# 3SAILab/two_stage_object_detection

Measured on AMD Instinct MI355X. Metric: images/sec Faster R-CNN ResNet-50 @800x1333, higher is better.
Workload: dtype f32 storage/accumulate; conv products as bf16x3 (3 exact bf16 pieces per operand, 6 bf16 MFMAs per product) in 0 of 43 conv layers, as fp16x2 (2 fp16 pieces of 2^e x per operand, 3 fp16 MFMAs per product; e follows the tensor's abs-max per forward: range words) in 43, f32 MFMA in the rest; 1 GPU; Full Faster R-CNN resnet50 inference forward, batch=1 per GPU, 3x800x1333, 80+1 classes, 3000->300 proposals; global_batch=1, parallelism=dp1, hip_graph=True, autotuned_tiles=True, steps_in_flight=4, tiles_tuned_on=this rank

## Files before the change

### two_stage_object_detection_amd/csrc/bottleneck_fused.hip

```cpp
#include "tsod_internal.h"
#include <type_traits>

namespace {

typedef float f32x16 __attribute__((ext_vector_type(16)));
typedef unsigned int u32x4 __attribute__((ext_vector_type(4)));

constexpr int TW = 16, HW_ = TW + 2;
constexpr int CMID = 64;
constexpr int Y_PITCH = 144;
constexpr int W_STEP = 8192;
template <int TH> struct Geo {
    static constexpr int HALO = (TH + 2) * (TW + 2);
    static constexpr int PB1 = (HALO + 31) / 32, PB2 = TH * TW / 32;
    static constexpr int Y_PLANE = PB1 * 32 * Y_PITCH;
    static constexpr int A_PLANE = PB1 * 32 * 64, A_STAGE = 2 * A_PLANE;
    static constexpr int Y_BYTES = 2 * Y_PLANE, SCR_OFF = Y_BYTES, LDS_BYTES = SCR_OFF + 64;
    static_assert(TH * TW % 32 == 0 && 2 * A_STAGE <= Y_BYTES && 2 * LDS_BYTES <= 160 * 1024, "x stages inside the y region; two workgroups per CU");
};
constexpr unsigned kOOB = 0xFFFFFFF0u;

struct Params {
    const float *x;
    float *out;
    const unsigned char *wstream;
    const float *bn;
    int N, H, W, Cin, in_pitch, Cout, out_pitch;
    int tiles_x, tiles_y;
    unsigned x_bytes, out_bytes;
    float slope;
    int w_exp1, w_exp2, w_exp3;
    float a_scale;
    const unsigned *amax_in;
    unsigned *amax_out;
    int *range_flag;
};

__device__ __forceinline__ int off64(int row, int slot) { return row * 64 + ((slot ^ ((row >> 2) & 3)) << 4); }

__device__ __forceinline__ float4 bload4(__amdgpu_buffer_rsrc_t r, unsigned off) {
    const u32x4 v = __builtin_amdgcn_raw_buffer_load_b128(r, off, 0, 0);
    return make_float4(__uint_as_float(v.x), __uint_as_float(v.y), __uint_as_float(v.z), __uint_as_float(v.w));
}

struct WFrag { u32x4 h[2], l[2]; };
struct AFrag { u32x4 h, l; };

template <int TH, bool PROJ = false>
__global__ void __launch_bounds__(256, 2) bottleneck_kernel(const Params p) {
    using G = Geo<TH>;
    constexpr int HALO = G::HALO, PB1 = G::PB1, PB2 = G::PB2, Y_PLANE = G::Y_PLANE, A_PLANE = G::A_PLANE, A_STAGE = G::A_STAGE,
                  SCR_OFF = G::SCR_OFF, LDS_BYTES = G::LDS_BYTES;
    __shared__ __align__(16) unsigned char lds[LDS_BYTES];
    const int tid = threadIdx.x, lane = tid & 63, wave = tid >> 6;
    const int j = lane & 31, hh = lane >> 5;
    const int cb = wave & 1, pb0 = wave >> 1;
    const int nb1 = (PB1 - pb0 + 1) / 2, nb2 = (PB2 - pb0 + 1) / 2;
    float *scr = reinterpret_cast<float *>(lds + SCR_OFF);

    const int tiles_per_img = p.tiles_x * p.tiles_y;
    const int nwg = (int)gridDim.x, per = nwg >> 3, r8 = nwg & 7, xcd = (int)blockIdx.x & 7;
    const int tile_id = (xcd < r8 ? xcd * (per + 1) : r8 * (per + 1) + (xcd - r8) * per) + ((int)blockIdx.x >> 3);
    const int img = tile_id / tiles_per_img, t_in = tile_id - img * tiles_per_img;
    const int ty = t_in / p.tiles_x, tx = t_in - ty * p.tiles_x;
    const int h0 = ty * TH, w0 = tx * TW;
    const __amdgpu_buffer_rsrc_t rs_x = __builtin_amdgcn_make_buffer_rsrc((void *)p.x, (short)0, (int)p.x_bytes, 0x00020000);
    const __amdgpu_buffer_rsrc_t rs_o = __builtin_amdgcn_make_buffer_rsrc((void *)p.out, (short)0, (int)p.out_bytes, 0x00020000);

    float a_scale = p.a_scale;
    int e_x;
    if (p.amax_in != nullptr) {
        e_x = tsod_fp16x2_exp_from_bits(tsod_amax_reduce_bits(p.amax_in[lane * TSOD_AMAX_STRIDE_WORDS]));
        a_scale = __uint_as_float((unsigned)(127 + e_x) << 23);
    } else {
        e_x = (int)(__float_as_uint(a_scale) >> 23) - 127;
    }
    a_scale = __uint_as_float((unsigned)__builtin_amdgcn_readfirstlane((int)__float_as_uint(a_scale)));

    const int n_steps1 = p.Cin / 32, sps = PROJ ? 2 + n_steps1 : 2, n_steps = n_steps1 + 18 + (p.Cout / 64) * sps;
    const u32x4 *wbase = reinterpret_cast<const u32x4 *>(p.wstream + cb * (W_STEP / 2) + lane * 64);
    auto w_load = [&](int s, WFrag &f) {
        if (s >= n_steps) return;
        const u32x4 *src = wbase + (size_t)s * (W_STEP / 16);
        f.h[0] = src[0]; f.l[0] = src[1]; f.h[1] = src[2]; f.l[1] = src[3];
    };
    WFrag wf[3];
    w_load(0, wf[0]);
    w_load(1, wf[1]);

    constexpr int NX = PB1;
    unsigned xoff[NX];
    int xdst[NX];
#pragma unroll
    for (int i = 0; i < NX; ++i) {
        const int u = tid + 256 * i, row = u >> 3, q = u & 7;
        const int hr = row / HW_, hc = row - hr * HW_;
        const int gh = h0 - 1 + hr, gw = w0 - 1 + hc;
        const bool ok = row < HALO && (unsigned)gh < (unsigned)p.H && (unsigned)gw < (unsigned)p.W;
        xoff[i] = ok ? (unsigned)((((long)img * p.H + gh) * p.W + gw) * p.in_pitch + q * 4) * 4u : kOOB;
        xdst[i] = off64(row, q >> 1) + (q & 1) * 8;
    }
    float4 xr[NX];
    auto x_load = [&](int ks) {
        if (ks >= n_steps1) return;
#pragma unroll
        for (int i = 0; i < NX; ++i) xr[i] = bload4(rs_x, xoff[i] != kOOB ? xoff[i] + (unsigned)ks * 128u : kOOB);
    };
    auto x_store = [&](int stage) {
#pragma unroll
        for (int i = 0; i < NX; ++i) {
            unsigned h0_, l0_, h1_, l1_;
            tsod_split2_pair(xr[i].x, xr[i].y, a_scale, h0_, l0_);
            tsod_split2_pair(xr[i].z, xr[i].w, a_scale, h1_, l1_);
            *reinterpret_cast<uint2 *>(lds + stage * A_STAGE + xdst[i]) = make_uint2(h0_, h1_);
            *reinterpret_cast<uint2 *>(lds + stage * A_STAGE + A_PLANE + xdst[i]) = make_uint2(l0_, l1_);
        }
    };
    int xfa[4][2];
#pragma unroll
    for (int b = 0; b < 4; ++b)
#pragma unroll
        for (int c = 0; c < 2; ++c) xfa[b][c] = off64((pb0 + 2 * b) * 32 + j, 2 * c + hh);

    f32x16 acc[4];
#pragma unroll
    for (int b = 0; b < 4; ++b)
#pragma unroll
        for (int e = 0; e < 16; ++e) acc[b][e] = 0.f;
    x_load(0);
    x_store(0);
    x_load(1);
    __syncthreads();
    auto conv1_step = [&](auto STAGE, int ks) {
        constexpr int stage = decltype(STAGE)::value;
        w_load(ks + 2, wf[2]);
        if (ks + 1 < n_steps1) x_store(stage ^ 1);
        x_load(ks + 2);
#pragma unroll
        for (int c = 0; c < 2; ++c) {
#pragma unroll
            for (int b = 0; b < 4; ++b) {
                if (b < nb1) {
                    const u32x4 ah = *reinterpret_cast<const u32x4 *>(lds + xfa[b][c] + stage * A_STAGE);
                    const u32x4 al = *reinterpret_cast<const u32x4 *>(lds + xfa[b][c] + stage * A_STAGE + A_PLANE);
                    tsod_mfma3(acc[b], wf[0].h[c], wf[0].l[c], ah, al);
                }
            }
        }
        wf[0] = wf[1];
        wf[1] = wf[2];
        __syncthreads();
    };
    for (int ks = 0; ks < n_steps1; ks += 2) {
        conv1_step(std::integral_constant<int, 0>{}, ks);
        conv1_step(std::integral_constant<int, 1>{}, ks + 1);
    }
    const int ch16 = cb * 32 + 16 * hh;
    const float sc1 = __uint_as_float((unsigned)(127 - e_x - p.w_exp1) << 23);
    float mx = 0.f, chk = 0.f;
    {
        float sv[16], bv[16];
#pragma unroll
        for (int v = 0; v < 4; ++v) {
            const float4 s4 = *reinterpret_cast<const float4 *>(p.bn + ch16 + 4 * v), b4 = *reinterpret_cast<const float4 *>(p.bn + 64 + ch16 + 4 * v);
            sv[4 * v] = s4.x * sc1; sv[4 * v + 1] = s4.y * sc1; sv[4 * v + 2] = s4.z * sc1; sv[4 * v + 3] = s4.w * sc1;
            bv[4 * v] = b4.x; bv[4 * v + 1] = b4.y; bv[4 * v + 2] = b4.z; bv[4 * v + 3] = b4.w;
        }
#pragma unroll
        for (int b = 0; b < 4; ++b) {
            if (b >= nb1) continue;
            const int row = (pb0 + 2 * b) * 32 + j, hr = row / HW_, hc = row - hr * HW_;
            const bool ok = row < HALO && (unsigned)(h0 - 1 + hr) < (unsigned)p.H && (unsigned)(w0 - 1 + hc) < (unsigned)p.W;
            const float keep = ok ? 1.f : 0.f;
#pragma unroll
            for (int e = 0; e < 16; ++e) {
                chk = fmaf(acc[b][e], 0.f, chk);
                const float v = keep * tsod_prelu(fmaf(acc[b][e], sv[e], bv[e]), p.slope);
                acc[b][e] = v;
                mx = fmaxf(mx, fabsf(v));
            }
        }
    }
    mx = tsod_block_max(mx, scr, tid);
    const int e1 = tsod_fp16x2_exp_from_bits(__float_as_uint(mx));
    const float ys1 = __uint_as_float((unsigned)(127 + e1) << 23);
    auto y_store = [&](const f32x16 &v, int row, float ysc) {
        unsigned hq[8], lq[8];
#pragma unroll
        for (int e = 0; e < 8; ++e) tsod_split2_pair(v[2 * e], v[2 * e + 1], ysc, hq[e], lq[e]);
        unsigned char *dst = lds + (row * Y_PITCH + (4 * cb + 2 * hh) * 16);
        *reinterpret_cast<u32x4 *>(dst) = u32x4{hq[0], hq[1], hq[2], hq[3]};
        *reinterpret_cast<u32x4 *>(dst + 16) = u32x4{hq[4], hq[5], hq[6], hq[7]};
        *reinterpret_cast<u32x4 *>(dst + Y_PLANE) = u32x4{lq[0], lq[1], lq[2], lq[3]};
        *reinterpret_cast<u32x4 *>(dst + Y_PLANE + 16) = u32x4{lq[4], lq[5], lq[6], lq[7]};
    };
#pragma unroll
    for (int b = 0; b < 4; ++b)
        if (b < nb1) y_store(acc[b], (pb0 + 2 * b) * 32 + j, ys1);
    __syncthreads();

    int yfa[3];
#pragma unroll
    for (int b = 0; b < 3; ++b) {
        int pidx = (pb0 + 2 * b) * 32 + j;
        pidx = pidx < TH * TW ? pidx : TH * TW - 1;
        yfa[b] = ((pidx / TW) * HW_ + (pidx % TW)) * Y_PITCH + hh * 16;
    }
#pragma unroll
    for (int b = 0; b < 3; ++b)
#pragma unroll
        for (int e = 0; e < 16; ++e) acc[b][e] = 0.f;
    const int s2base = n_steps1;
    AFrag af[2][3];
    auto y1_frags = [&](int n, AFrag (&f)[3]) {
        const int t = n >> 1, c = n & 1, tap = t >> 1, kh = tap / 3, kw = tap - kh * 3;
        const int imm = (kh * HW_ + kw) * Y_PITCH + (t & 1) * 64 + c * 32;
#pragma unroll
        for (int b = 0; b < 3; ++b)
            if (b < nb2) {
                f[b].h = *reinterpret_cast<const u32x4 *>(lds + yfa[b] + imm);
                f[b].l = *reinterpret_cast<const u32x4 *>(lds + yfa[b] + imm + Y_PLANE);
            }
    };
    y1_frags(0, af[0]);
#pragma unroll
    for (int t = 0; t < 18; ++t) {
        w_load(s2base + t + 2, wf[(t + 2) % 3]);
#pragma unroll
        for (int c = 0; c < 2; ++c) {
            const int n = 2 * t + c;
            if (n + 1 < 36) y1_frags(n + 1, af[(n + 1) & 1]);
#pragma unroll
            for (int b = 0; b < 3; ++b)
                if (b < nb2) tsod_mfma3(acc[b], wf[t % 3].h[c], wf[t % 3].l[c], af[n & 1][b].h, af[n & 1][b].l);
            __builtin_amdgcn_sched_barrier(0);
        }
    }
    __syncthreads();
    const float sc2 = __uint_as_float((unsigned)(127 - e1 - p.w_exp2) << 23);
    mx = 0.f;
    {
        float sv[16], bv[16];
#pragma unroll
        for (int v = 0; v < 4; ++v) {
            const float4 s4 = *reinterpret_cast<const float4 *>(p.bn + 128 + ch16 + 4 * v), b4 = *reinterpret_cast<const float4 *>(p.bn + 192 + ch16 + 4 * v);
            sv[4 * v] = s4.x * sc2; sv[4 * v + 1] = s4.y * sc2; sv[4 * v + 2] = s4.z * sc2; sv[4 * v + 3] = s4.w * sc2;
            bv[4 * v] = b4.x; bv[4 * v + 1] = b4.y; bv[4 * v + 2] = b4.z; bv[4 * v + 3] = b4.w;
        }
#pragma unroll
        for (int b = 0; b < 3; ++b) {
            if (b >= nb2) continue;
#pragma unroll
            for (int e = 0; e < 16; ++e) {
                chk = fmaf(acc[b][e], 0.f, chk);
                const float v = tsod_prelu(fmaf(acc[b][e], sv[e], bv[e]), p.slope);
                acc[b][e] = v;
                mx = fmaxf(mx, fabsf(v));
            }
        }
    }
    mx = tsod_block_max(mx, scr, tid);
    const int e2 = tsod_fp16x2_exp_from_bits(__float_as_uint(mx));
    const float ys2 = __uint_as_float((unsigned)(127 + e2) << 23);
#pragma unroll
    for (int b = 0; b < 3; ++b)
        if (b < nb2) y_store(acc[b], (pb0 + 2 * b) * 32 + j, ys2);
    __syncthreads();

    const float sc3 = __uint_as_float((unsigned)(127 - e2 - p.w_exp3) << 23);
    float amax = 0.f;
    constexpr int P_PITCH = 144, P_BYTES = 32 * P_PITCH;
    static_assert(2 * P_BYTES <= Y_PLANE - TH * TW * Y_PITCH, "two patches per gap of the y region");
    unsigned char *patch = lds + (wave >> 1) * Y_PLANE + TH * TW * Y_PITCH + (wave & 1) * P_BYTES;
    const int ep_px = lane >> 3, ep_q = lane & 7;
    int y2a[3];
    unsigned xpix[3][4], opix[3][4];
#pragma unroll
    for (int b = 0; b < 3; ++b) {
        const int pidx = (pb0 + 2 * b) * 32 + j;
        y2a[b] = (pidx < TH * TW ? pidx : TH * TW - 1) * Y_PITCH + hh * 16;
#pragma unroll
        for (int i = 0; i < 4; ++i) {
            const int pe = (pb0 + 2 * b) * 32 + ep_px + 8 * i, pr = pe >> 4, pc = pe & 15;
            const bool ok = b < nb2 && pe < TH * TW && h0 + pr < p.H && w0 + pc < p.W;
            const long gp = ((long)img * p.H + h0 + pr) * p.W + w0 + pc;
            xpix[b][i] = ok ? (unsigned)(gp * p.in_pitch + cb * 32 + ep_q * 4) * 4u : kOOB;
            opix[b][i] = ok ? (unsigned)(gp * p.out_pitch + cb * 32 + ep_q * 4) * 4u : kOOB;
        }
    }
    static_assert(TW == 16 && (PB1 + 1) / 2 <= 4 && (PB2 + 1) / 2 <= 3, "pixel index -> (row, column) by shifts; blocks per wave");
    auto y2_frags = [&](int n, AFrag (&f)[3]) {
#pragma unroll
        for (int b = 0; b < 3; ++b)
            if (b < nb2) {
                f[b].h = *reinterpret_cast<const u32x4 *>(lds + y2a[b] + n * 32);
                f[b].l = *reinterpret_cast<const u32x4 *>(lds + y2a[b] + n * 32 + Y_PLANE);
            }
    };
    const int s3base = n_steps1 + 18;
  if constexpr (PROJ) {
    unsigned xfo[3];
#pragma unroll
    for (int b = 0; b < 3; ++b) {
        const int pidx = (pb0 + 2 * b) * 32 + j, pr = pidx >> 4, pc = pidx & 15;
        const bool ok = b < nb2 && pidx < TH * TW && h0 + pr < p.H && w0 + pc < p.W;
        xfo[b] = ok ? (unsigned)((((long)img * p.H + h0 + pr) * p.W + w0 + pc) * p.in_pitch + 8 * hh) * 4u : kOOB;
    }
    const float rescale = __uint_as_float((unsigned)(127 + e_x - e2) << 23);
    const float sc3x = __uint_as_float((unsigned)(127 - e_x - p.w_exp3) << 23);
    float4 xraw[2][3][2];
    auto x_frag_load = [&](int xs) {
#pragma unroll
        for (int c = 0; c < 2; ++c)
#pragma unroll
            for (int b = 0; b < 3; ++b) {
                const unsigned o = xfo[b] != kOOB ? xfo[b] + (unsigned)(32 * xs + 16 * c) * 4u : kOOB;
                xraw[c][b][0] = bload4(rs_x, o);
                xraw[c][b][1] = bload4(rs_x, o != kOOB ? o + 16u : kOOB);
            }
    };
    for (int q = 0; q < p.Cout / 64; ++q) {
#pragma unroll
        for (int b = 0; b < 3; ++b)
#pragma unroll
            for (int e = 0; e < 16; ++e) acc[b][e] = 0.f;
        const unsigned chq = (unsigned)(q * 64) * 4u;
        const int sbase = s3base + q * sps;
        for (int st = 0; st < sps; ++st) {
            w_load(sbase + st + 2, wf[2]);
            if (st < 2) {
                if (st == 1) x_frag_load(0);
#pragma unroll
                for (int c = 0; c < 2; ++c) {
                    y2_frags(2 * st + c, af[c]);
#pragma unroll
                    for (int b = 0; b < 3; ++b)
                        if (b < nb2) tsod_mfma3(acc[b], wf[0].h[c], wf[0].l[c], af[c][b].h, af[c][b].l);
                }
                if (st == 1) {
#pragma unroll
                    for (int b = 0; b < 3; ++b)
#pragma unroll
                        for (int e = 0; e < 16; ++e) acc[b][e] *= rescale;
                }
            } else {
#pragma unroll
                for (int c = 0; c < 2; ++c)
#pragma unroll
                    for (int b = 0; b < 3; ++b) {
                        unsigned h0_, l0_, h1_, l1_, h2_, l2_, h3_, l3_;
                        tsod_split2_pair(xraw[c][b][0].x, xraw[c][b][0].y, a_scale, h0_, l0_);
                        tsod_split2_pair(xraw[c][b][0].z, xraw[c][b][0].w, a_scale, h1_, l1_);
                        tsod_split2_pair(xraw[c][b][1].x, xraw[c][b][1].y, a_scale, h2_, l2_);
                        tsod_split2_pair(xraw[c][b][1].z, xraw[c][b][1].w, a_scale, h3_, l3_);
                        af[c][b].h = u32x4{h0_, h1_, h2_, h3_};
                        af[c][b].l = u32x4{l0_, l1_, l2_, l3_};
                    }
                if (st + 1 < sps) x_frag_load(st - 1);
#pragma unroll
                for (int c = 0; c < 2; ++c)
#pragma unroll
                    for (int b = 0; b < 3; ++b)
                        if (b < nb2) tsod_mfma3(acc[b], wf[0].h[c], wf[0].l[c], af[c][b].h, af[c][b].l);
            }
            wf[0] = wf[1];
            wf[1] = wf[2];
        }
        const float4 s4 = *reinterpret_cast<const float4 *>(p.bn + 256 + q * 64 + cb * 32 + ep_q * 4);
        const float4 b4 = *reinterpret_cast<const float4 *>(p.bn + 256 + p.Cout + q * 64 + cb * 32 + ep_q * 4);
        const float4 sv = make_float4(s4.x * sc3x, s4.y * sc3x, s4.z * sc3x, s4.w * sc3x);
#pragma unroll
        for (int b = 0; b < 3; ++b) {
            if (b >= nb2) continue;
#pragma unroll
            for (int v = 0; v < 4; ++v) {
                chk = fmaf(acc[b][4 * v], 0.f, fmaf(acc[b][4 * v + 1], 0.f, fmaf(acc[b][4 * v + 2], 0.f, fmaf(acc[b][4 * v + 3], 0.f, chk))));
                *reinterpret_cast<float4 *>(patch + j * P_PITCH + (16 * hh + 4 * v) * 4) =
                    make_float4(acc[b][4 * v], acc[b][4 * v + 1], acc[b][4 * v + 2], acc[b][4 * v + 3]);
            }
            asm volatile("s_waitcnt lgkmcnt(0)" ::: "memory");
            float4 t[4];
#pragma unroll
            for (int i = 0; i < 4; ++i) t[i] = *reinterpret_cast<const float4 *>(patch + (ep_px + 8 * i) * P_PITCH + ep_q * 16);
            asm volatile("s_waitcnt lgkmcnt(0)" ::: "memory");
            float m4 = 0.f;
#pragma unroll
            for (int i = 0; i < 4; ++i) {
                const float o0 = tsod_prelu(fmaf(t[i].x, sv.x, b4.x), p.slope);
                const float o1 = tsod_prelu(fmaf(t[i].y, sv.y, b4.y), p.slope);
                const float o2 = tsod_prelu(fmaf(t[i].z, sv.z, b4.z), p.slope);
                const float o3 = tsod_prelu(fmaf(t[i].w, sv.w, b4.w), p.slope);
                const float m = fmaxf(fmaxf(fabsf(o0), fabsf(o1)), fmaxf(fabsf(o2), fabsf(o3)));
                m4 = fmaxf(m4, opix[b][i] != kOOB ? m : 0.f);
                u32x4 o;
                o.x = __float_as_uint(o0); o.y = __float_as_uint(o1); o.z = __float_as_uint(o2); o.w = __float_as_uint(o3);
                __builtin_amdgcn_raw_buffer_store_b128(o, rs_o, opix[b][i] != kOOB ? opix[b][i] + chq : kOOB, 0, 0);
            }
            amax = fmaxf(amax, m4);
        }
    }
  } else {
      for (int q = 0; q < p.Cout / 64; ++q) {
  #pragma unroll
          for (int b = 0; b < 3; ++b)
  #pragma unroll
              for (int e = 0; e < 16; ++e) acc[b][e] = 0.f;
          const unsigned chq = (unsigned)(q * 64) * 4u;
          w_load(s3base + 2 * q + 2, wf[2]);
          float4 res[3][4];
  #pragma unroll
          for (int b = 0; b < 3; ++b)
  #pragma unroll
              for (int i = 0; i < 4; ++i) res[b][i] = bload4(rs_x, xpix[b][i] != kOOB ? xpix[b][i] + chq : kOOB);
          y2_frags(0, af[0]);
  #pragma unroll
          for (int n = 0; n < 4; ++n) {
              if (n == 2) w_load(s3base + 2 * q + 3, wf[0]);
              if (n + 1 < 4) y2_frags(n + 1, af[(n + 1) & 1]);
  #pragma unroll
              for (int b = 0; b < 3; ++b)
                  if (b < nb2) tsod_mfma3(acc[b], wf[n >> 1].h[n & 1], wf[n >> 1].l[n & 1], af[n & 1][b].h, af[n & 1][b].l);
              __builtin_amdgcn_sched_barrier(0);
          }
          const float4 s4 = *reinterpret_cast<const float4 *>(p.bn + 256 + q * 64 + cb * 32 + ep_q * 4);
          const float4 b4 = *reinterpret_cast<const float4 *>(p.bn + 256 + p.Cout + q * 64 + cb * 32 + ep_q * 4);
          const float4 sv = make_float4(s4.x * sc3, s4.y * sc3, s4.z * sc3, s4.w * sc3);
  #pragma unroll
          for (int b = 0; b < 3; ++b) {
              if (b >= nb2) continue;
  #pragma unroll
              for (int v = 0; v < 4; ++v) {
                  chk = fmaf(acc[b][4 * v], 0.f, fmaf(acc[b][4 * v + 1], 0.f, fmaf(acc[b][4 * v + 2], 0.f, fmaf(acc[b][4 * v + 3], 0.f, chk))));
                  *reinterpret_cast<float4 *>(patch + j * P_PITCH + (16 * hh + 4 * v) * 4) =
                      make_float4(acc[b][4 * v], acc[b][4 * v + 1], acc[b][4 * v + 2], acc[b][4 * v + 3]);
              }
              asm volatile("s_waitcnt lgkmcnt(0)" ::: "memory");
              float4 t[4];
  #pragma unroll
              for (int i = 0; i < 4; ++i) t[i] = *reinterpret_cast<const float4 *>(patch + (ep_px + 8 * i) * P_PITCH + ep_q * 16);
              asm volatile("s_waitcnt lgkmcnt(0)" ::: "memory");
              float m4 = 0.f;
  #pragma unroll
              for (int i = 0; i < 4; ++i) {
                  const float o0 = tsod_prelu(fmaf(t[i].x, sv.x, b4.x + res[b][i].x), p.slope);
                  const float o1 = tsod_prelu(fmaf(t[i].y, sv.y, b4.y + res[b][i].y), p.slope);
                  const float o2 = tsod_prelu(fmaf(t[i].z, sv.z, b4.z + res[b][i].z), p.slope);
                  const float o3 = tsod_prelu(fmaf(t[i].w, sv.w, b4.w + res[b][i].w), p.slope);
                  const float m = fmaxf(fmaxf(fabsf(o0), fabsf(o1)), fmaxf(fabsf(o2), fabsf(o3)));
                  m4 = fmaxf(m4, opix[b][i] != kOOB ? m : 0.f);
                  u32x4 o;
                  o.x = __float_as_uint(o0); o.y = __float_as_uint(o1); o.z = __float_as_uint(o2); o.w = __float_as_uint(o3);
                  __builtin_amdgcn_raw_buffer_store_b128(o, rs_o, opix[b][i] != kOOB ? opix[b][i] + chq : kOOB, 0, 0);
              }
              amax = fmaxf(amax, m4);
          }
          wf[1] = wf[0];
          wf[0] = wf[2];
      }
  }
    if (p.range_flag != nullptr && __any(!(chk == 0.f)) && lane == 0) atomicOr(p.range_flag, 1);
    if (p.amax_out != nullptr) tsod_amax_commit(p.amax_out, amax, scr, tid, 256);
}

}

extern "C" size_t tsod_bottleneck_wstream_bytes(int32_t Cin, int32_t Cout) {
    if (Cin <= 0 || Cout <= 0 || Cin % 32 || Cout % 64) return 0;
    return (size_t)(Cin / 32 + 18 + (Cout / 64) * 2) * W_STEP;
}

extern "C" size_t tsod_bottleneck_proj_wstream_bytes(int32_t Cin, int32_t Cout) {
    if (Cin <= 0 || Cout <= 0 || Cin % 64 || Cout % 64) return 0;
    return (size_t)(Cin / 32 + 18 + (Cout / 64) * (2 + Cin / 32)) * W_STEP;
}

extern "C" int tsod_bottleneck_fp16x2(const tsod_bottleneck_desc *d, const float *x, const void *wstream, const float *bn,
                                      float *out, tsod_stream_t stream) {
    TSOD_REQUIRE(d && x && wstream && bn && out, TSOD_ERR_INVALID_ARG);
    TSOD_REQUIRE(d->N > 0 && d->H > 0 && d->W > 0, TSOD_ERR_INVALID_ARG);
    TSOD_REQUIRE(d->projection == 0 || d->projection == 1, TSOD_ERR_INVALID_ARG);
    const bool proj = d->projection == 1;
    TSOD_REQUIRE(d->Cmid == CMID && d->Cin % 32 == 0 && d->Cin >= 32 && d->Cout % 64 == 0 && (proj || d->Cout == d->Cin), TSOD_ERR_UNSUPPORTED);
    TSOD_REQUIRE(d->in_pitch >= d->Cin && d->out_pitch >= d->Cout && (d->in_pitch & 3) == 0 && (d->out_pitch & 3) == 0, TSOD_ERR_ALIGNMENT);
    TSOD_REQUIRE(tsod_aligned16(x) && tsod_aligned16(out) && tsod_aligned16(wstream) && tsod_aligned16(bn), TSOD_ERR_ALIGNMENT);
    TSOD_REQUIRE((reinterpret_cast<uintptr_t>(d->amax_in) & 63u) == 0 && (reinterpret_cast<uintptr_t>(d->amax_out) & 63u) == 0, TSOD_ERR_ALIGNMENT);
    TSOD_REQUIRE(d->a_scale_exp >= -24 && d->a_scale_exp <= 24, TSOD_ERR_INVALID_ARG);
    TSOD_REQUIRE((uint64_t)d->N * d->H * d->W * d->in_pitch * 4 < 0xFFFFFFF0ull, TSOD_ERR_UNSUPPORTED);
    Params p;
    p.x = x; p.out = out; p.wstream = static_cast<const unsigned char *>(wstream); p.bn = bn;
    p.N = d->N; p.H = d->H; p.W = d->W; p.Cin = d->Cin; p.in_pitch = d->in_pitch; p.Cout = d->Cout; p.out_pitch = d->out_pitch;
    int cus = 0, dev = 0;
    if (hipGetDevice(&dev) != hipSuccess || hipDeviceGetAttribute(&cus, hipDeviceAttributeMultiprocessorCount, dev) != hipSuccess || cus <= 0) {
        (void)hipGetLastError();
        cus = 256;
    }
    auto cost = [&](int th, int mfma_slowest) {
        const int64_t tiles = (int64_t)d->N * ((d->W + TW - 1) / TW) * ((d->H + th - 1) / th);
        return (double)((tiles + 2 * cus - 1) / (2 * cus)) * mfma_slowest;
    };
    const int n1 = d->Cin / 32, nq = d->Cout / 64, c3 = proj ? 4 + 2 * n1 : 4;
    const int TH = cost(8, 3 * (3 * 2 * n1 + 2 * 36 + 2 * c3 * nq)) < cost(10, 3 * (4 * 2 * n1 + 3 * 36 + 3 * c3 * nq)) ? 8 : 10;
    p.tiles_x = (d->W + TW - 1) / TW; p.tiles_y = (d->H + TH - 1) / TH;
    TSOD_REQUIRE((uint64_t)d->N * d->H * d->W * d->out_pitch * 4 < 0xFFFFFFF0ull && d->Cin % 64 == 0, TSOD_ERR_UNSUPPORTED);
    p.x_bytes = (unsigned)((uint64_t)d->N * d->H * d->W * d->in_pitch * 4);
    p.out_bytes = (unsigned)((uint64_t)d->N * d->H * d->W * d->out_pitch * 4);
    p.slope = d->slope; p.w_exp1 = d->w_exp[0]; p.w_exp2 = d->w_exp[1]; p.w_exp3 = d->w_exp[2];
    p.a_scale = ldexpf(1.f, d->a_scale_exp);
    p.amax_in = d->amax_in; p.amax_out = d->amax_out; p.range_flag = d->range_flag;
    const int64_t grid = (int64_t)d->N * p.tiles_x * p.tiles_y;
    TSOD_REQUIRE(grid < 0x7FFFFFFF, TSOD_ERR_UNSUPPORTED);
    if (proj) {
        if (TH == 8) hipLaunchKernelGGL((bottleneck_kernel<8, true>), dim3((unsigned)grid), dim3(256), 0, tsod_stream(stream), p);
        else hipLaunchKernelGGL((bottleneck_kernel<10, true>), dim3((unsigned)grid), dim3(256), 0, tsod_stream(stream), p);
    } else {
        if (TH == 8) hipLaunchKernelGGL((bottleneck_kernel<8, false>), dim3((unsigned)grid), dim3(256), 0, tsod_stream(stream), p);
        else hipLaunchKernelGGL((bottleneck_kernel<10, false>), dim3((unsigned)grid), dim3(256), 0, tsod_stream(stream), p);
    }
    return tsod_launch_status();
}
```

Measured before the change: 1189 images/s.

## Run TH=8 bottleneck tiles at three workgroups per CU with compact LDS

Adds a WPC template parameter so the TH=8 fused bottleneck kernel targets three workgroups per CU. It shrinks the y region, swizzles the epilogue patch with a 128-byte pitch, and skips storing conv1 halo padding rows. The change also moves weight loads to buffer loads with immediate offsets, replaces per-element address arrays with a shared pixel index plus computed offsets to save registers, and uses a swizzle-based block max. Tile height selection now models three slots per CU for TH=8, which favours smaller tiles. The tighter register budget risks spills, and the higher occupancy trades against fewer fragments in flight per wave.

```diff
diff --git a/two_stage_object_detection_amd/csrc/bottleneck_fused.hip b/two_stage_object_detection_amd/csrc/bottleneck_fused.hip
--- a/two_stage_object_detection_amd/csrc/bottleneck_fused.hip
+++ b/two_stage_object_detection_amd/csrc/bottleneck_fused.hip
@@ -10,13 +10,17 @@
 constexpr int CMID = 64;
 constexpr int Y_PITCH = 144;
 constexpr int W_STEP = 8192;
-template <int TH> struct Geo {
+template <int TH, int WPC> struct Geo {
     static constexpr int HALO = (TH + 2) * (TW + 2);
     static constexpr int PB1 = (HALO + 31) / 32, PB2 = TH * TW / 32;
-    static constexpr int Y_PLANE = PB1 * 32 * Y_PITCH;
+    static constexpr int NB1 = (PB1 + 1) / 2, NB2 = (PB2 + 1) / 2;
+    static constexpr int P_PITCH = WPC == 3 ? 128 : Y_PITCH, P_BYTES = 32 * P_PITCH;
+    static constexpr int Y_PLANE = WPC == 3 ? TH * TW * Y_PITCH + 2 * P_BYTES : PB1 * 32 * Y_PITCH;
     static constexpr int A_PLANE = PB1 * 32 * 64, A_STAGE = 2 * A_PLANE;
     static constexpr int Y_BYTES = 2 * Y_PLANE, SCR_OFF = Y_BYTES, LDS_BYTES = SCR_OFF + 64;
     static_assert(TH * TW % 32 == 0 && 2 * A_STAGE <= Y_BYTES && 2 * LDS_BYTES <= 160 * 1024, "x stages inside the y region; two workgroups per CU");
+    static_assert(WPC == 2 || (WPC == 3 && 3 * LDS_BYTES <= 160 * 1024 && PB1 % 2 == 0 && PB2 % 2 == 0), "three workgroups per CU: 54 613 bytes each, even block counts");
+    static_assert(HALO * Y_PITCH <= Y_PLANE && TH * TW * Y_PITCH + 2 * P_BYTES <= Y_PLANE, "a plane holds y1's halo rows, and y2's rows + two patches");
 };
 constexpr unsigned kOOB = 0xFFFFFFF0u;
 
@@ -43,19 +47,32 @@
     return make_float4(__uint_as_float(v.x), __uint_as_float(v.y), __uint_as_float(v.z), __uint_as_float(v.w));
 }
 
+__device__ __forceinline__ float block_max_imm(float v, float *scr, int tid) {
+    v = fmaxf(v, __int_as_float(__builtin_amdgcn_ds_swizzle(__float_as_int(v), 0x041F)));
+    v = fmaxf(v, __int_as_float(__builtin_amdgcn_ds_swizzle(__float_as_int(v), 0x081F)));
+    v = fmaxf(v, __int_as_float(__builtin_amdgcn_ds_swizzle(__float_as_int(v), 0x101F)));
+    v = fmaxf(v, __int_as_float(__builtin_amdgcn_ds_swizzle(__float_as_int(v), 0x201F)));
+    v = fmaxf(v, __int_as_float(__builtin_amdgcn_ds_swizzle(__float_as_int(v), 0x401F)));
+    v = fmaxf(__int_as_float(__builtin_amdgcn_readlane(__float_as_int(v), 0)), __int_as_float(__builtin_amdgcn_readlane(__float_as_int(v), 32)));
+    __syncthreads();
+    if ((tid & 63) == 0) scr[tid >> 6] = v;
+    __syncthreads();
+    return fmaxf(fmaxf(scr[0], scr[1]), fmaxf(scr[2], scr[3]));
+}
+
 struct WFrag { u32x4 h[2], l[2]; };
 struct AFrag { u32x4 h, l; };
 
-template <int TH, bool PROJ = false>
-__global__ void __launch_bounds__(256, 2) bottleneck_kernel(const Params p) {
-    using G = Geo<TH>;
-    constexpr int HALO = G::HALO, PB1 = G::PB1, PB2 = G::PB2, Y_PLANE = G::Y_PLANE, A_PLANE = G::A_PLANE, A_STAGE = G::A_STAGE,
-                  SCR_OFF = G::SCR_OFF, LDS_BYTES = G::LDS_BYTES;
-    __shared__ __align__(16) unsigned char lds[LDS_BYTES];
+template <int TH, bool PROJ, int WPC>
+__global__ void __launch_bounds__(256, WPC) bottleneck_kernel(const Params p) {
+    using G = Geo<TH, WPC>;
+    constexpr int HALO = G::HALO, PB1 = G::PB1, PB2 = G::PB2, NB1 = G::NB1, NB2 = G::NB2, Y_PLANE = G::Y_PLANE, A_PLANE = G::A_PLANE,
+                  A_STAGE = G::A_STAGE, SCR_OFF = G::SCR_OFF, LDS_BYTES = G::LDS_BYTES;
+    __shared__ __align__(128) unsigned char lds[LDS_BYTES];
     const int tid = threadIdx.x, lane = tid & 63, wave = tid >> 6;
     const int j = lane & 31, hh = lane >> 5;
     const int cb = wave & 1, pb0 = wave >> 1;
-    const int nb1 = (PB1 - pb0 + 1) / 2, nb2 = (PB2 - pb0 + 1) / 2;
+    const int nb1 = PB1 % 2 == 0 ? PB1 / 2 : (PB1 - pb0 + 1) / 2, nb2 = PB2 % 2 == 0 ? PB2 / 2 : (PB2 - pb0 + 1) / 2;
     float *scr = reinterpret_cast<float *>(lds + SCR_OFF);
 
     const int tiles_per_img = p.tiles_x * p.tiles_y;
@@ -78,11 +95,14 @@
     a_scale = __uint_as_float((unsigned)__builtin_amdgcn_readfirstlane((int)__float_as_uint(a_scale)));
 
     const int n_steps1 = p.Cin / 32, sps = PROJ ? 2 + n_steps1 : 2, n_steps = n_steps1 + 18 + (p.Cout / 64) * sps;
-    const u32x4 *wbase = reinterpret_cast<const u32x4 *>(p.wstream + cb * (W_STEP / 2) + lane * 64);
+    const __amdgpu_buffer_rsrc_t rs_w = __builtin_amdgcn_make_buffer_rsrc((void *)p.wstream, (short)0, n_steps * W_STEP, 0x00020000);
+    const unsigned woff = (unsigned)(cb * (W_STEP / 2) + lane * 64);
     auto w_load = [&](int s, WFrag &f) {
         if (s >= n_steps) return;
-        const u32x4 *src = wbase + (size_t)s * (W_STEP / 16);
-        f.h[0] = src[0]; f.l[0] = src[1]; f.h[1] = src[2]; f.l[1] = src[3];
+        f.h[0] = __builtin_amdgcn_raw_buffer_load_b128(rs_w, woff, s * W_STEP, 0);
+        f.l[0] = __builtin_amdgcn_raw_buffer_load_b128(rs_w, woff + 16u, s * W_STEP, 0);
+        f.h[1] = __builtin_amdgcn_raw_buffer_load_b128(rs_w, woff + 32u, s * W_STEP, 0);
+        f.l[1] = __builtin_amdgcn_raw_buffer_load_b128(rs_w, woff + 48u, s * W_STEP, 0);
     };
     WFrag wf[3];
     w_load(0, wf[0]);
@@ -90,15 +110,14 @@
 
     constexpr int NX = PB1;
     unsigned xoff[NX];
-    int xdst[NX];
+    const int xdst = off64(tid >> 3, (tid & 7) >> 1) + (tid & 1) * 8;
 #pragma unroll
     for (int i = 0; i < NX; ++i) {
         const int u = tid + 256 * i, row = u >> 3, q = u & 7;
         const int hr = row / HW_, hc = row - hr * HW_;
         const int gh = h0 - 1 + hr, gw = w0 - 1 + hc;
         const bool ok = row < HALO && (unsigned)gh < (unsigned)p.H && (unsigned)gw < (unsigned)p.W;
-        xoff[i] = ok ? (unsigned)((((long)img * p.H + gh) * p.W + gw) * p.in_pitch + q * 4) * 4u : kOOB;
-        xdst[i] = off64(row, q >> 1) + (q & 1) * 8;
+        xoff[i] = ok ? ((unsigned)((img * p.H + gh) * p.W + gw) * (unsigned)p.in_pitch + q * 4) * 4u : kOOB;
     }
     float4 xr[NX];
     auto x_load = [&](int ks) {
@@ -112,19 +131,17 @@
             unsigned h0_, l0_, h1_, l1_;
             tsod_split2_pair(xr[i].x, xr[i].y, a_scale, h0_, l0_);
             tsod_split2_pair(xr[i].z, xr[i].w, a_scale, h1_, l1_);
-            *reinterpret_cast<uint2 *>(lds + stage * A_STAGE + xdst[i]) = make_uint2(h0_, h1_);
-            *reinterpret_cast<uint2 *>(lds + stage * A_STAGE + A_PLANE + xdst[i]) = make_uint2(l0_, l1_);
-        }
-    };
-    int xfa[4][2];
-#pragma unroll
-    for (int b = 0; b < 4; ++b)
-#pragma unroll
-        for (int c = 0; c < 2; ++c) xfa[b][c] = off64((pb0 + 2 * b) * 32 + j, 2 * c + hh);
-
-    f32x16 acc[4];
-#pragma unroll
-    for (int b = 0; b < 4; ++b)
+            *reinterpret_cast<uint2 *>(lds + stage * A_STAGE + 2048 * i + xdst) = make_uint2(h0_, h1_);
+            *reinterpret_cast<uint2 *>(lds + stage * A_STAGE + A_PLANE + 2048 * i + xdst) = make_uint2(l0_, l1_);
+        }
+    };
+    int xfa[2];
+    xfa[0] = off64(pb0 * 32 + j, hh);
+    xfa[1] = xfa[0] ^ 32;
+
+    f32x16 acc[NB1];
+#pragma unroll
+    for (int b = 0; b < NB1; ++b)
 #pragma unroll
         for (int e = 0; e < 16; ++e) acc[b][e] = 0.f;
     x_load(0);
@@ -139,10 +156,10 @@
 #pragma unroll
         for (int c = 0; c < 2; ++c) {
 #pragma unroll
-            for (int b = 0; b < 4; ++b) {
+            for (int b = 0; b < NB1; ++b) {
                 if (b < nb1) {
-                    const u32x4 ah = *reinterpret_cast<const u32x4 *>(lds + xfa[b][c] + stage * A_STAGE);
-                    const u32x4 al = *reinterpret_cast<const u32x4 *>(lds + xfa[b][c] + stage * A_STAGE + A_PLANE);
+                    const u32x4 ah = *reinterpret_cast<const u32x4 *>(lds + xfa[c] + 4096 * b + stage * A_STAGE);
+                    const u32x4 al = *reinterpret_cast<const u32x4 *>(lds + xfa[c] + 4096 * b + stage * A_STAGE + A_PLANE);
                     tsod_mfma3(acc[b], wf[0].h[c], wf[0].l[c], ah, al);
                 }
             }
@@ -167,7 +184,7 @@
             bv[4 * v] = b4.x; bv[4 * v + 1] = b4.y; bv[4 * v + 2] = b4.z; bv[4 * v + 3] = b4.w;
         }
 #pragma unroll
-        for (int b = 0; b < 4; ++b) {
+        for (int b = 0; b < NB1; ++b) {
             if (b >= nb1) continue;
             const int row = (pb0 + 2 * b) * 32 + j, hr = row / HW_, hc = row - hr * HW_;
             const bool ok = row < HALO && (unsigned)(h0 - 1 + hr) < (unsigned)p.H && (unsigned)(w0 - 1 + hc) < (unsigned)p.W;
@@ -181,13 +198,14 @@
             }
         }
     }
-    mx = tsod_block_max(mx, scr, tid);
+    mx = block_max_imm(mx, scr, tid);
     const int e1 = tsod_fp16x2_exp_from_bits(__float_as_uint(mx));
     const float ys1 = __uint_as_float((unsigned)(127 + e1) << 23);
     auto y_store = [&](const f32x16 &v, int row, float ysc) {
         unsigned hq[8], lq[8];
 #pragma unroll
         for (int e = 0; e < 8; ++e) tsod_split2_pair(v[2 * e], v[2 * e + 1], ysc, hq[e], lq[e]);
+        if (WPC == 3 && row >= HALO) return;
         unsigned char *dst = lds + (row * Y_PITCH + (4 * cb + 2 * hh) * 16);
         *reinterpret_cast<u32x4 *>(dst) = u32x4{hq[0], hq[1], hq[2], hq[3]};
         *reinterpret_cast<u32x4 *>(dst + 16) = u32x4{hq[4], hq[5], hq[6], hq[7]};
@@ -195,28 +213,28 @@
         *reinterpret_cast<u32x4 *>(dst + Y_PLANE + 16) = u32x4{lq[4], lq[5], lq[6], lq[7]};
     };
 #pragma unroll
-    for (int b = 0; b < 4; ++b)
+    for (int b = 0; b < NB1; ++b)
         if (b < nb1) y_store(acc[b], (pb0 + 2 * b) * 32 + j, ys1);
     __syncthreads();
 
-    int yfa[3];
-#pragma unroll
-    for (int b = 0; b < 3; ++b) {
+    int yfa[NB2];
+#pragma unroll
+    for (int b = 0; b < NB2; ++b) {
         int pidx = (pb0 + 2 * b) * 32 + j;
         pidx = pidx < TH * TW ? pidx : TH * TW - 1;
         yfa[b] = ((pidx / TW) * HW_ + (pidx % TW)) * Y_PITCH + hh * 16;
     }
 #pragma unroll
-    for (int b = 0; b < 3; ++b)
+    for (int b = 0; b < NB2; ++b)
 #pragma unroll
         for (int e = 0; e < 16; ++e) acc[b][e] = 0.f;
     const int s2base = n_steps1;
-    AFrag af[2][3];
-    auto y1_frags = [&](int n, AFrag (&f)[3]) {
+    AFrag af[2][NB2];
+    auto y1_frags = [&](int n, AFrag (&f)[NB2]) {
         const int t = n >> 1, c = n & 1, tap = t >> 1, kh = tap / 3, kw = tap - kh * 3;
         const int imm = (kh * HW_ + kw) * Y_PITCH + (t & 1) * 64 + c * 32;
 #pragma unroll
-        for (int b = 0; b < 3; ++b)
+        for (int b = 0; b < NB2; ++b)
             if (b < nb2) {
                 f[b].h = *reinterpret_cast<const u32x4 *>(lds + yfa[b] + imm);
                 f[b].l = *reinterpret_cast<const u32x4 *>(lds + yfa[b] + imm + Y_PLANE);
@@ -231,7 +249,7 @@
             const int n = 2 * t + c;
             if (n + 1 < 36) y1_frags(n + 1, af[(n + 1) & 1]);
 #pragma unroll
-            for (int b = 0; b < 3; ++b)
+            for (int b = 0; b < NB2; ++b)
                 if (b < nb2) tsod_mfma3(acc[b], wf[t % 3].h[c], wf[t % 3].l[c], af[n & 1][b].h, af[n & 1][b].l);
             __builtin_amdgcn_sched_barrier(0);
         }
@@ -248,7 +266,7 @@
             bv[4 * v] = b4.x; bv[4 * v + 1] = b4.y; bv[4 * v + 2] = b4.z; bv[4 * v + 3] = b4.w;
         }
 #pragma unroll
-        for (int b = 0; b < 3; ++b) {
+        for (int b = 0; b < NB2; ++b) {
             if (b >= nb2) continue;
 #pragma unroll
             for (int e = 0; e < 16; ++e) {
@@ -259,69 +277,85 @@
             }
         }
     }
-    mx = tsod_block_max(mx, scr, tid);
+    mx = block_max_imm(mx, scr, tid);
     const int e2 = tsod_fp16x2_exp_from_bits(__float_as_uint(mx));
     const float ys2 = __uint_as_float((unsigned)(127 + e2) << 23);
 #pragma unroll
-    for (int b = 0; b < 3; ++b)
+    for (int b = 0; b < NB2; ++b)
         if (b < nb2) y_store(acc[b], (pb0 + 2 * b) * 32 + j, ys2);
     __syncthreads();
 
     const float sc3 = __uint_as_float((unsigned)(127 - e2 - p.w_exp3) << 23);
     float amax = 0.f;
-    constexpr int P_PITCH = 144, P_BYTES = 32 * P_PITCH;
-    static_assert(2 * P_BYTES <= Y_PLANE - TH * TW * Y_PITCH, "two patches per gap of the y region");
-    unsigned char *patch = lds + (wave >> 1) * Y_PLANE + TH * TW * Y_PITCH + (wave & 1) * P_BYTES;
+    constexpr int P_PITCH = G::P_PITCH, P_BYTES = G::P_BYTES;
     const int ep_px = lane >> 3, ep_q = lane & 7;
-    int y2a[3];
-    unsigned xpix[3][4], opix[3][4];
-#pragma unroll
-    for (int b = 0; b < 3; ++b) {
+    const int patch = (wave >> 1) * Y_PLANE + TH * TW * Y_PITCH + (wave & 1) * P_BYTES;
+    const int patch_w = patch + j * P_PITCH + (WPC == 3 ? ((4 * hh) ^ (j & 7)) << 4 : hh * 64);
+    const int patch_r = patch + ep_px * P_PITCH + (WPC == 3 ? ep_q ^ ep_px : ep_q) * 16;
+    auto patch_put = [&](int v, float4 f) { *reinterpret_cast<float4 *>(lds + (WPC == 3 ? patch_w ^ (v << 4) : patch_w + v * 16)) = f; };
+    auto patch_get = [&](int i) { return *reinterpret_cast<const float4 *>(lds + patch_r + 8 * i * P_PITCH); };
+    int y2a[NB2];
+    unsigned epix[NB2][4];
+    const __amdgpu_buffer_rsrc_t rs_bn = __builtin_amdgcn_make_buffer_rsrc((void *)p.bn, (short)0, (256 + 2 * p.Cout) * 4, 0x00020000);
+    const unsigned ep_c = (unsigned)(cb * 32 + ep_q * 4) * 4u, x_pitch4 = (unsigned)p.in_pitch * 4u, o_pitch4 = (unsigned)p.out_pitch * 4u;
+#pragma unroll
+    for (int b = 0; b < NB2; ++b) {
         const int pidx = (pb0 + 2 * b) * 32 + j;
         y2a[b] = (pidx < TH * TW ? pidx : TH * TW - 1) * Y_PITCH + hh * 16;
 #pragma unroll
         for (int i = 0; i < 4; ++i) {
             const int pe = (pb0 + 2 * b) * 32 + ep_px + 8 * i, pr = pe >> 4, pc = pe & 15;
             const bool ok = b < nb2 && pe < TH * TW && h0 + pr < p.H && w0 + pc < p.W;
-            const long gp = ((long)img * p.H + h0 + pr) * p.W + w0 + pc;
-            xpix[b][i] = ok ? (unsigned)(gp * p.in_pitch + cb * 32 + ep_q * 4) * 4u : kOOB;
-            opix[b][i] = ok ? (unsigned)(gp * p.out_pitch + cb * 32 + ep_q * 4) * 4u : kOOB;
-        }
-    }
-    static_assert(TW == 16 && (PB1 + 1) / 2 <= 4 && (PB2 + 1) / 2 <= 3, "pixel index -> (row, column) by shifts; blocks per wave");
-    auto y2_frags = [&](int n, AFrag (&f)[3]) {
-#pragma unroll
-        for (int b = 0; b < 3; ++b)
+            epix[b][i] = ok ? (unsigned)((img * p.H + h0 + pr) * p.W + w0 + pc) : kOOB;
+        }
+    }
+    static_assert(TW == 16 && NB2 <= NB1, "pixel index -> (row, column) by shifts; conv2 and conv3 re-use conv1's accumulators");
+    constexpr int FG = WPC == 3 ? 1 : NB2, NG = NB2 / FG;
+    auto y2_frags = [&](int u, AFrag (&f)[NB2]) {
+#pragma unroll
+        for (int i = 0; i < FG; ++i) {
+            const int n = u / NG, b = (u % NG) * FG + i;
             if (b < nb2) {
-                f[b].h = *reinterpret_cast<const u32x4 *>(lds + y2a[b] + n * 32);
-                f[b].l = *reinterpret_cast<const u32x4 *>(lds + y2a[b] + n * 32 + Y_PLANE);
-            }
+                f[i].h = *reinterpret_cast<const u32x4 *>(lds + y2a[b] + n * 32);
+                f[i].l = *reinterpret_cast<const u32x4 *>(lds + y2a[b] + n * 32 + Y_PLANE);
+            }
+        }
     };
     const int s3base = n_steps1 + 18;
   if constexpr (PROJ) {
-    unsigned xfo[3];
-#pragma unroll
-    for (int b = 0; b < 3; ++b) {
+    unsigned xfo[NB2];
+#pragma unroll
+    for (int b = 0; b < NB2; ++b) {
         const int pidx = (pb0 + 2 * b) * 32 + j, pr = pidx >> 4, pc = pidx & 15;
         const bool ok = b < nb2 && pidx < TH * TW && h0 + pr < p.H && w0 + pc < p.W;
-        xfo[b] = ok ? (unsigned)((((long)img * p.H + h0 + pr) * p.W + w0 + pc) * p.in_pitch + 8 * hh) * 4u : kOOB;
+        xfo[b] = ok ? ((unsigned)((img * p.H + h0 + pr) * p.W + w0 + pc) * (unsigned)p.in_pitch + 8 * hh) * 4u : kOOB;
     }
     const float rescale = __uint_as_float((unsigned)(127 + e_x - e2) << 23);
     const float sc3x = __uint_as_float((unsigned)(127 - e_x - p.w_exp3) << 23);
-    float4 xraw[2][3][2];
+    float4 xraw[2][NB2][2];
+    auto x_frag_load_one = [&](int xs, int c, int b) {
+        const unsigned o = xfo[b] != kOOB ? xfo[b] + (unsigned)(32 * xs + 16 * c) * 4u : kOOB;
+        xraw[c][b][0] = bload4(rs_x, o);
+        xraw[c][b][1] = bload4(rs_x, o != kOOB ? o + 16u : kOOB);
+    };
     auto x_frag_load = [&](int xs) {
 #pragma unroll
         for (int c = 0; c < 2; ++c)
 #pragma unroll
-            for (int b = 0; b < 3; ++b) {
-                const unsigned o = xfo[b] != kOOB ? xfo[b] + (unsigned)(32 * xs + 16 * c) * 4u : kOOB;
-                xraw[c][b][0] = bload4(rs_x, o);
-                xraw[c][b][1] = bload4(rs_x, o != kOOB ? o + 16u : kOOB);
-            }
+            for (int b = 0; b < NB2; ++b) x_frag_load_one(xs, c, b);
+    };
+    auto x_split = [&](const float4 (&r)[2], AFrag &f) {
+        unsigned h0_, l0_, h1_, l1_, h2_, l2_, h3_, l3_;
+        tsod_split2_pair(r[0].x, r[0].y, a_scale, h0_, l0_);
+        tsod_split2_pair(r[0].z, r[0].w, a_scale, h1_, l1_);
+        tsod_split2_pair(r[1].x, r[1].y, a_scale, h2_, l2_);
+        tsod_split2_pair(r[1].z, r[1].w, a_scale, h3_, l3_);
+        f.h = u32x4{h0_, h1_, h2_, h3_};
+        f.l = u32x4{l0_, l1_, l2_, l3_};
     };
     for (int q = 0; q < p.Cout / 64; ++q) {
 #pragma unroll
-        for (int b = 0; b < 3; ++b)
+        for (int b = 0; b < NB2; ++b)
 #pragma unroll
             for (int e = 0; e < 16; ++e) acc[b][e] = 0.f;
         const unsigned chq = (unsigned)(q * 64) * 4u;
@@ -331,57 +365,60 @@
             if (st < 2) {
                 if (st == 1) x_frag_load(0);
 #pragma unroll
-                for (int c = 0; c < 2; ++c) {
-                    y2_frags(2 * st + c, af[c]);
-#pragma unroll
-                    for (int b = 0; b < 3; ++b)
-                        if (b < nb2) tsod_mfma3(acc[b], wf[0].h[c], wf[0].l[c], af[c][b].h, af[c][b].l);
-                }
+                for (int c = 0; c < 2; ++c)
+#pragma unroll
+                    for (int g = 0; g < NG; ++g) {
+                        const int u = c * NG + g;
+                        y2_frags(2 * st * NG + u, af[u & 1]);
+#pragma unroll
+                        for (int i = 0; i < FG; ++i)
+                            if (g * FG + i < nb2) tsod_mfma3(acc[g * FG + i], wf[0].h[c], wf[0].l[c], af[u & 1][i].h, af[u & 1][i].l);
+                    }
                 if (st == 1) {
 #pragma unroll
-                    for (int b = 0; b < 3; ++b)
+                    for (int b = 0; b < NB2; ++b)
 #pragma unroll
                         for (int e = 0; e < 16; ++e) acc[b][e] *= rescale;
                 }
+            } else if constexpr (WPC == 3) {
+#pragma unroll
+                for (int c = 0; c < 2; ++c)
+#pragma unroll
+                    for (int b = 0; b < NB2; ++b) {
+                        AFrag &f = af[b & 1][0];
+                        x_split(xraw[c][b], f);
+                        if (st + 1 < sps) x_frag_load_one(st - 1, c, b);
+                        tsod_mfma3(acc[b], wf[0].h[c], wf[0].l[c], f.h, f.l);
+                    }
             } else {
 #pragma unroll
                 for (int c = 0; c < 2; ++c)
 #pragma unroll
-                    for (int b = 0; b < 3; ++b) {
-                        unsigned h0_, l0_, h1_, l1_, h2_, l2_, h3_, l3_;
-                        tsod_split2_pair(xraw[c][b][0].x, xraw[c][b][0].y, a_scale, h0_, l0_);
-                        tsod_split2_pair(xraw[c][b][0].z, xraw[c][b][0].w, a_scale, h1_, l1_);
-                        tsod_split2_pair(xraw[c][b][1].x, xraw[c][b][1].y, a_scale, h2_, l2_);
-                        tsod_split2_pair(xraw[c][b][1].z, xraw[c][b][1].w, a_scale, h3_, l3_);
-                        af[c][b].h = u32x4{h0_, h1_, h2_, h3_};
-                        af[c][b].l = u32x4{l0_, l1_, l2_, l3_};
-                    }
+                    for (int b = 0; b < NB2; ++b) x_split(xraw[c][b], af[c][b]);
                 if (st + 1 < sps) x_frag_load(st - 1);
 #pragma unroll
                 for (int c = 0; c < 2; ++c)
 #pragma unroll
-                    for (int b = 0; b < 3; ++b)
+                    for (int b = 0; b < NB2; ++b)
                         if (b < nb2) tsod_mfma3(acc[b], wf[0].h[c], wf[0].l[c], af[c][b].h, af[c][b].l);
             }
             wf[0] = wf[1];
             wf[1] = wf[2];
         }
-        const float4 s4 = *reinterpret_cast<const float4 *>(p.bn + 256 + q * 64 + cb * 32 + ep_q * 4);
-        const float4 b4 = *reinterpret_cast<const float4 *>(p.bn + 256 + p.Cout + q * 64 + cb * 32 + ep_q * 4);
+        const float4 s4 = bload4(rs_bn, ep_c + (unsigned)(256 + q * 64) * 4u), b4 = bload4(rs_bn, ep_c + (unsigned)(256 + p.Cout + q * 64) * 4u);
         const float4 sv = make_float4(s4.x * sc3x, s4.y * sc3x, s4.z * sc3x, s4.w * sc3x);
 #pragma unroll
-        for (int b = 0; b < 3; ++b) {
+        for (int b = 0; b < NB2; ++b) {
             if (b >= nb2) continue;
 #pragma unroll
             for (int v = 0; v < 4; ++v) {
                 chk = fmaf(acc[b][4 * v], 0.f, fmaf(acc[b][4 * v + 1], 0.f, fmaf(acc[b][4 * v + 2], 0.f, fmaf(acc[b][4 * v + 3], 0.f, chk))));
-                *reinterpret_cast<float4 *>(patch + j * P_PITCH + (16 * hh + 4 * v) * 4) =
-                    make_float4(acc[b][4 * v], acc[b][4 * v + 1], acc[b][4 * v + 2], acc[b][4 * v + 3]);
+                patch_put(v, make_float4(acc[b][4 * v], acc[b][4 * v + 1], acc[b][4 * v + 2], acc[b][4 * v + 3]));
             }
             asm volatile("s_waitcnt lgkmcnt(0)" ::: "memory");
             float4 t[4];
 #pragma unroll
-            for (int i = 0; i < 4; ++i) t[i] = *reinterpret_cast<const float4 *>(patch + (ep_px + 8 * i) * P_PITCH + ep_q * 16);
+            for (int i = 0; i < 4; ++i) t[i] = patch_get(i);
             asm volatile("s_waitcnt lgkmcnt(0)" ::: "memory");
             float m4 = 0.f;
 #pragma unroll
@@ -391,10 +428,10 @@
                 const float o2 = tsod_prelu(fmaf(t[i].z, sv.z, b4.z), p.slope);
                 const float o3 = tsod_prelu(fmaf(t[i].w, sv.w, b4.w), p.slope);
                 const float m = fmaxf(fmaxf(fabsf(o0), fabsf(o1)), fmaxf(fabsf(o2), fabsf(o3)));
-                m4 = fmaxf(m4, opix[b][i] != kOOB ? m : 0.f);
+                m4 = fmaxf(m4, epix[b][i] != kOOB ? m : 0.f);
                 u32x4 o;
                 o.x = __float_as_uint(o0); o.y = __float_as_uint(o1); o.z = __float_as_uint(o2); o.w = __float_as_uint(o3);
-                __builtin_amdgcn_raw_buffer_store_b128(o, rs_o, opix[b][i] != kOOB ? opix[b][i] + chq : kOOB, 0, 0);
+                __builtin_amdgcn_raw_buffer_store_b128(o, rs_o, epix[b][i] != kOOB ? epix[b][i] * o_pitch4 + ep_c + chq : kOOB, 0, 0);
             }
             amax = fmaxf(amax, m4);
         }
@@ -402,42 +439,43 @@
   } else {
       for (int q = 0; q < p.Cout / 64; ++q) {
   #pragma unroll
-          for (int b = 0; b < 3; ++b)
+          for (int b = 0; b < NB2; ++b)
   #pragma unroll
               for (int e = 0; e < 16; ++e) acc[b][e] = 0.f;
           const unsigned chq = (unsigned)(q * 64) * 4u;
           w_load(s3base + 2 * q + 2, wf[2]);
-          float4 res[3][4];
-  #pragma unroll
-          for (int b = 0; b < 3; ++b)
-  #pragma unroll
-              for (int i = 0; i < 4; ++i) res[b][i] = bload4(rs_x, xpix[b][i] != kOOB ? xpix[b][i] + chq : kOOB);
+          float4 res[NB2][4];
+  #pragma unroll
+          for (int b = 0; b < NB2; ++b)
+  #pragma unroll
+              for (int i = 0; i < 4; ++i) res[b][i] = bload4(rs_x, epix[b][i] != kOOB ? epix[b][i] * x_pitch4 + ep_c + chq : kOOB);
           y2_frags(0, af[0]);
   #pragma unroll
-          for (int n = 0; n < 4; ++n) {
-              if (n == 2) w_load(s3base + 2 * q + 3, wf[0]);
-              if (n + 1 < 4) y2_frags(n + 1, af[(n + 1) & 1]);
-  #pragma unroll
-              for (int b = 0; b < 3; ++b)
-                  if (b < nb2) tsod_mfma3(acc[b], wf[n >> 1].h[n & 1], wf[n >> 1].l[n & 1], af[n & 1][b].h, af[n & 1][b].l);
+          for (int u = 0; u < 4 * NG; ++u) {
+              const int n = u / NG;
+              if (u == 2 * NG) w_load(s3base + 2 * q + 3, wf[0]);
+              if (u + 1 < 4 * NG) y2_frags(u + 1, af[(u + 1) & 1]);
+  #pragma unroll
+              for (int i = 0; i < FG; ++i) {
+                  const int b = (u % NG) * FG + i;
+                  if (b < nb2) tsod_mfma3(acc[b], wf[n >> 1].h[n & 1], wf[n >> 1].l[n & 1], af[u & 1][i].h, af[u & 1][i].l);
+              }
               __builtin_amdgcn_sched_barrier(0);
           }
-          const float4 s4 = *reinterpret_cast<const float4 *>(p.bn + 256 + q * 64 + cb * 32 + ep_q * 4);
-          const float4 b4 = *reinterpret_cast<const float4 *>(p.bn + 256 + p.Cout + q * 64 + cb * 32 + ep_q * 4);
+          const float4 s4 = bload4(rs_bn, ep_c + (unsigned)(256 + q * 64) * 4u), b4 = bload4(rs_bn, ep_c + (unsigned)(256 + p.Cout + q * 64) * 4u);
           const float4 sv = make_float4(s4.x * sc3, s4.y * sc3, s4.z * sc3, s4.w * sc3);
   #pragma unroll
-          for (int b = 0; b < 3; ++b) {
+          for (int b = 0; b < NB2; ++b) {
               if (b >= nb2) continue;
   #pragma unroll
               for (int v = 0; v < 4; ++v) {
                   chk = fmaf(acc[b][4 * v], 0.f, fmaf(acc[b][4 * v + 1], 0.f, fmaf(acc[b][4 * v + 2], 0.f, fmaf(acc[b][4 * v + 3], 0.f, chk))));
-                  *reinterpret_cast<float4 *>(patch + j * P_PITCH + (16 * hh + 4 * v) * 4) =
-                      make_float4(acc[b][4 * v], acc[b][4 * v + 1], acc[b][4 * v + 2], acc[b][4 * v + 3]);
+                  patch_put(v, make_float4(acc[b][4 * v], acc[b][4 * v + 1], acc[b][4 * v + 2], acc[b][4 * v + 3]));
               }
               asm volatile("s_waitcnt lgkmcnt(0)" ::: "memory");
               float4 t[4];
   #pragma unroll
-              for (int i = 0; i < 4; ++i) t[i] = *reinterpret_cast<const float4 *>(patch + (ep_px + 8 * i) * P_PITCH + ep_q * 16);
+              for (int i = 0; i < 4; ++i) t[i] = patch_get(i);
               asm volatile("s_waitcnt lgkmcnt(0)" ::: "memory");
               float m4 = 0.f;
   #pragma unroll
@@ -447,10 +485,10 @@
                   const float o2 = tsod_prelu(fmaf(t[i].z, sv.z, b4.z + res[b][i].z), p.slope);
                   const float o3 = tsod_prelu(fmaf(t[i].w, sv.w, b4.w + res[b][i].w), p.slope);
                   const float m = fmaxf(fmaxf(fabsf(o0), fabsf(o1)), fmaxf(fabsf(o2), fabsf(o3)));
-                  m4 = fmaxf(m4, opix[b][i] != kOOB ? m : 0.f);
+                  m4 = fmaxf(m4, epix[b][i] != kOOB ? m : 0.f);
                   u32x4 o;
                   o.x = __float_as_uint(o0); o.y = __float_as_uint(o1); o.z = __float_as_uint(o2); o.w = __float_as_uint(o3);
-                  __builtin_amdgcn_raw_buffer_store_b128(o, rs_o, opix[b][i] != kOOB ? opix[b][i] + chq : kOOB, 0, 0);
+                  __builtin_amdgcn_raw_buffer_store_b128(o, rs_o, epix[b][i] != kOOB ? epix[b][i] * o_pitch4 + ep_c + chq : kOOB, 0, 0);
               }
               amax = fmaxf(amax, m4);
           }
@@ -494,12 +532,12 @@
         (void)hipGetLastError();
         cus = 256;
     }
-    auto cost = [&](int th, int mfma_slowest) {
-        const int64_t tiles = (int64_t)d->N * ((d->W + TW - 1) / TW) * ((d->H + th - 1) / th);
-        return (double)((tiles + 2 * cus - 1) / (2 * cus)) * mfma_slowest;
+    auto cost = [&](int th, int wpc, int mfma_slowest) {
+        const int64_t tiles = (int64_t)d->N * ((d->W + TW - 1) / TW) * ((d->H + th - 1) / th), slots = (int64_t)wpc * cus;
+        return (double)((tiles + slots - 1) / slots) * mfma_slowest;
     };
     const int n1 = d->Cin / 32, nq = d->Cout / 64, c3 = proj ? 4 + 2 * n1 : 4;
-    const int TH = cost(8, 3 * (3 * 2 * n1 + 2 * 36 + 2 * c3 * nq)) < cost(10, 3 * (4 * 2 * n1 + 3 * 36 + 3 * c3 * nq)) ? 8 : 10;
+    const int TH = cost(8, 3, 3 * (3 * 2 * n1 + 2 * 36 + 2 * c3 * nq)) < cost(10, 2, 3 * (4 * 2 * n1 + 3 * 36 + 3 * c3 * nq)) ? 8 : 10;
     p.tiles_x = (d->W + TW - 1) / TW; p.tiles_y = (d->H + TH - 1) / TH;
     TSOD_REQUIRE((uint64_t)d->N * d->H * d->W * d->out_pitch * 4 < 0xFFFFFFF0ull && d->Cin % 64 == 0, TSOD_ERR_UNSUPPORTED);
     p.x_bytes = (unsigned)((uint64_t)d->N * d->H * d->W * d->in_pitch * 4);
@@ -509,12 +547,9 @@
     p.amax_in = d->amax_in; p.amax_out = d->amax_out; p.range_flag = d->range_flag;
     const int64_t grid = (int64_t)d->N * p.tiles_x * p.tiles_y;
     TSOD_REQUIRE(grid < 0x7FFFFFFF, TSOD_ERR_UNSUPPORTED);
-    if (proj) {
-        if (TH == 8) hipLaunchKernelGGL((bottleneck_kernel<8, true>), dim3((unsigned)grid), dim3(256), 0, tsod_stream(stream), p);
-        else hipLaunchKernelGGL((bottleneck_kernel<10, true>), dim3((unsigned)grid), dim3(256), 0, tsod_stream(stream), p);
-    } else {
-        if (TH == 8) hipLaunchKernelGGL((bottleneck_kernel<8, false>), dim3((unsigned)grid), dim3(256), 0, tsod_stream(stream), p);
-        else hipLaunchKernelGGL((bottleneck_kernel<10, false>), dim3((unsigned)grid), dim3(256), 0, tsod_stream(stream), p);
-    }
+    void (*kernel)(const Params);
+    if (proj) kernel = TH == 10 ? bottleneck_kernel<10, true, 2> : bottleneck_kernel<8, true, 3>;
+    else kernel = TH == 10 ? bottleneck_kernel<10, false, 2> : bottleneck_kernel<8, false, 3>;
+    hipLaunchKernelGGL(kernel, dim3((unsigned)grid), dim3(256), 0, tsod_stream(stream), p);
     return tsod_launch_status();
 }
```

Result: faster. 1205 images/s, median of 6 (+1.3%).
